# dhansmair/flamingo-mini

Measured on AMD Instinct MI355X. Metric: images/sec (fwd+bwd) flamingo-mini bs=32, higher is better.
Workload: dtype bf16

## Files before the change

### flamingo-mini_amd/build.py

```python
from __future__ import annotations

import concurrent.futures
import os
import shutil
import subprocess
import sys

PKG_DIR = os.path.dirname(os.path.abspath(__file__))
CSRC = os.path.join(PKG_DIR, "csrc")
LIB_PATH = os.path.join(PKG_DIR, "libflamingo_fusion.so")
SOURCES = ["ff_api.hip", "ff_gemm.hip", "ff_rowwise.hip", "ff_attention.hip", "ff_xattn_fused.hip", "ff_optim.hip", "ff_loss.hip", "ff_elementwise.hip", "ff_decode.hip", "ff_sample.hip", "ff_beam.hip", "ff_logits.hip", "ff_logprob.hip", "ff_constrain.hip", "ff_guidance.hip", "ff_truncate.hip", "ff_score.hip", "ff_beam_sample.hip", "ff_contrastive.hip"]
HEADERS = ["ff_common.h", "ff_internal.h", "ff_gemm_tiles.h", "ff_attention_core.h", "ff_row_keys.h", "ff_sr.h", "ff_beam_walk.h", os.path.join("..", "..", "include", "flamingo_fusion.h")]
ARCH = "gfx950"
FLAGS = [f"--offload-arch={ARCH}", "-O3", "-std=c++17", "-fPIC", "-fvisibility=hidden", "-Wno-unused-result", "-mllvm", "-amdgpu-kernarg-preload-count=16"] + os.environ.get("FF_EXTRA_FLAGS", "").split()


def _hipcc() -> str:
    for cand in (os.environ.get("HIPCC"), "/opt/rocm/bin/hipcc", shutil.which("hipcc")):
        if cand and os.path.exists(cand):
            return cand
    raise RuntimeError("hipcc not found (needs ROCm >= 7.0 for gfx950)")


def _stale(target: str, deps) -> bool:
    if not os.path.exists(target):
        return True
    t = os.path.getmtime(target)
    return any(os.path.getmtime(d) > t for d in deps)


def build(force: bool = False, verbose: bool = False, debug: bool = False) -> str:
    hipcc = _hipcc()
    obj_dir = os.path.join(CSRC, "_obj_debug" if debug else "_obj")
    lib_path = LIB_PATH.replace(".so", "_debug.so") if debug else LIB_PATH
    flags = FLAGS + (["-DFF_DEBUG"] if debug else [])
    os.makedirs(obj_dir, exist_ok=True)
    headers = [os.path.normpath(os.path.join(CSRC, h)) for h in HEADERS]
    jobs = []
    for src in SOURCES:
        s = os.path.join(CSRC, src)
        o = os.path.join(obj_dir, src.replace(".hip", ".o"))
        if force or _stale(o, [s] + headers) or not os.path.exists(o.replace(".o", ".resources.txt")):
            jobs.append((s, o))

    def compile_one(job):
        s, o = job
        cmd = [hipcc] + flags + ["-Rpass-analysis=kernel-resource-usage", "-c", s, "-o", o]
        r = subprocess.run(cmd, capture_output=True, text=True)
        if r.returncode != 0:
            raise RuntimeError(f"hipcc failed for {s}:\n{r.stderr[-4000:]}")
        with open(o.replace(".o", ".resources.txt"), "w") as f:
            f.write("\n".join(l for l in r.stderr.splitlines() if "kernel-resource-usage" in l) + "\n")
        if verbose:
            print("compiled", os.path.basename(s))
        return o

    with concurrent.futures.ThreadPoolExecutor(max_workers=len(SOURCES)) as ex:
        list(ex.map(compile_one, jobs))
    objs = [os.path.join(obj_dir, s.replace(".hip", ".o")) for s in SOURCES]
    if force or jobs or _stale(lib_path, objs + [os.path.join(CSRC, "exports.map")]):
        r = subprocess.run([hipcc, f"--offload-arch={ARCH}", "-shared", "-fPIC", f"-Wl,--version-script={os.path.join(CSRC, 'exports.map')}", "-o", lib_path] + objs,
                           capture_output=True, text=True)
        if r.returncode != 0:
            raise RuntimeError(f"link failed:\n{r.stderr[-4000:]}")
# ... 8 lines not shown
```

### flamingo-mini_amd/ffi.py

```python
from __future__ import annotations

import ctypes as C
import os
from typing import Optional, Sequence

import torch

PKG_DIR = os.path.dirname(os.path.abspath(__file__))
_which = os.environ.get("FLAMINGO_FUSION_LIB", "")
LIB_PATH = os.path.join(PKG_DIR, "libflamingo_fusion_debug.so") if _which == "debug" else (_which or os.path.join(PKG_DIR, "libflamingo_fusion.so"))
ABI_VERSION = 6

FF_OK = 0
DTYPE_F32, DTYPE_BF16 = 0, 1
ACT_NONE, ACT_GELU, ACT_SQRELU, ACT_RELU = -1, 0, 1, 2
ACTS = {"gelu": ACT_GELU, "sqrelu": ACT_SQRELU, "relu": ACT_RELU}
ATTN_DENSE, ATTN_MEDIA = 0, 1
RESAMPLER_GLOBAL_PARAMS, RESAMPLER_LAYER_PARAMS, XATTN_PARAMS = 4, 12, 11
XA_SAVED = {"mean_a": 0, "rstd_a": 1, "yn": 2, "y1": 3, "mean_f": 4, "rstd_f": 5, "xn_f": 6}
XA_SAVED_STAGES = {"Qs": 7, "lse": 8, "O": 9, "attn_out": 10, "Hpre": 11, "Aact": 12, "ffw_out": 13}
XA_SAVED_ORDER = ("mean_a", "rstd_a", "yn", "Qs", "lse", "O", "attn_out", "y1", "mean_f", "rstd_f", "xn_f", "Hpre", "Aact", "ffw_out")
XA_STASH = {"dy1": 0, "dH": 1, "dQs": 2}
WGRAD_GROUP_MAX = 12

# ... 81 lines not shown
    _fields_ = [(n, C.c_int) for n in ("dtype", "b", "k", "dim")] + [("ld_hidden", C.c_longlong)] + \
               [(n, C.c_int) for n in ("max_len", "eos", "pad", "reserved")] + \
               [(n, C.c_void_p) for n in ("hidden", "hist", "mask", "cand_tok", "cand_logp", "finished", "next_tok", "logprob", "sel_row", "beam_idx", "score")]


_P, _SZ, _I = C.c_void_p, C.c_size_t, C.c_int
_SIGNATURES = {
    "ff_version": (_I, []),
    "ff_arch": (C.c_char_p, []),
    "ff_last_error": (C.c_char_p, []),
    "ff_gemm_workspace_bytes": (_SZ, [C.POINTER(GemmDesc)]),
    "ff_gemm": (_I, [C.POINTER(GemmDesc), _P, _P, _P, _P, _P, _P, _P, _P, _SZ, _P]),
    "ff_gemm_profile_enable": (_I, [_I]),
    "ff_gemm_profile_read": (_I, [C.POINTER(GemmProfileRecord), _I]),
    "ff_gemm_plan": (_I, [C.POINTER(GemmDesc), C.POINTER(_I), C.POINTER(_I), C.POINTER(_I)]),
    "ff_layernorm_fwd": (_I, [C.POINTER(LnDesc), _P, _P, _P, _P, _P, _P, _P, _P]),
    "ff_layernorm_bwd_workspace_bytes": (_SZ, [C.POINTER(LnDesc)]),
    "ff_layernorm_bwd": (_I, [C.POINTER(LnDesc), _P, _P, _P, _P, _P, _P, _P, _P, _P, _P, _P, _SZ, _P]),
    "ff_rows_reduce_workspace_bytes": (_SZ, [C.POINTER(ReduceDesc)]),
    "ff_rows_reduce": (_I, [C.POINTER(ReduceDesc), _P, _P, _P, _SZ, _P]),
    "ff_gate_grad_workspace_bytes": (_SZ, [_I, _I]),
    "ff_gate_grad": (_I, [_I, _I, _I, _P, _P, _P, _P, _P, _SZ, _P]),
    "ff_text_time": (_I, [_I, _I, _P, _I, _P, _P]),
    "ff_attention_fwd": (_I, [C.POINTER(AttnDesc), _P, _P, _P, _P, _P, _P, _P]),
    "ff_attention_bwd_workspace_bytes": (_SZ, [C.POINTER(AttnDesc)]),
    "ff_attention_bwd": (_I, [C.POINTER(AttnDesc), _P, _P, _P, _P, _P, _P, _P, _P, _P, _P, _P, _SZ, _P]),
    "ff_resampler_saved_bytes": (_SZ, [C.POINTER(ResamplerDesc)]),
    "ff_resampler_scratch_bytes": (_SZ, [C.POINTER(ResamplerDesc)]),
    "ff_resampler_fwd": (_I, [C.POINTER(ResamplerDesc), _P, _P, _P, _P, _SZ, _P, _SZ, _P]),
    "ff_resampler_bwd": (_I, [C.POINTER(ResamplerDesc), _P, _P, _P, _P, _SZ, _P, _P, _P, _SZ, _P]),
    "ff_resampler_prologue_saved_bytes": (_SZ, [C.POINTER(ResamplerDesc)]),
    "ff_resampler_layer_saved_bytes": (_SZ, [C.POINTER(ResamplerDesc)]),
    "ff_resampler_layer_scratch_bytes": (_SZ, [C.POINTER(ResamplerDesc)]),
    "ff_resampler_epilogue_saved_bytes": (_SZ, [C.POINTER(ResamplerDesc)]),
    "ff_resampler_prologue_fwd": (_I, [C.POINTER(ResamplerDesc), _P, _P, _P, _SZ, _P]),
    "ff_resampler_layer_fwd": (_I, [C.POINTER(ResamplerDesc), _P, _P, _P, _SZ, _P, _I, _P, _P, _P, _SZ, _P, _SZ, _P]),
    "ff_resampler_epilogue_fwd": (_I, [C.POINTER(ResamplerDesc), _P, _P, _P, _P, _P, _SZ, _P]),
    "ff_resampler_epilogue_bwd": (_I, [C.POINTER(ResamplerDesc), _P, _P, _P, _P, _SZ, _P, _P, _P, _P, _SZ, _P]),
    "ff_resampler_layer_bwd": (_I, [C.POINTER(ResamplerDesc), _P, _P, _P, _SZ, _P, _I, _P, _P, _P, _SZ, _P, _P, _P, _I, _P, _SZ, _P]),
    "ff_resampler_prologue_bwd": (_I, [C.POINTER(ResamplerDesc), _P, _P, _P, _P, _P, _SZ, _P]),
    "ff_xattn_sync_bytes": (_SZ, []),
    "ff_xattn_sync_status": (_I, [_P, _P]),
    "ff_xattn_saved_bytes": (_SZ, [C.POINTER(XattnDesc)]),
    "ff_xattn_scratch_bytes": (_SZ, [C.POINTER(XattnDesc)]),
    "ff_xattn_kv_offset": (_SZ, [C.POINTER(XattnDesc)]),
    "ff_xattn_saved_view": (_I, [C.POINTER(XattnDesc), _I, C.POINTER(_SZ), C.POINTER(_SZ)]),
    "ff_xattn_block_fwd": (_I, [C.POINTER(XattnDesc), _P, _P, _P, _P, _P, _P, _P, _P, _SZ, _P, _SZ, _P]),
    "ff_quick_gelu_fwd": (_I, [_I, C.c_longlong, _P, _P, _P]),
    "ff_quick_gelu_bwd": (_I, [_I, C.c_longlong, _P, _P, _P, _P]),
    "ff_shifted_ce_fwd": (_I, [_I, _I, _I, _I, _P, _P, C.c_longlong, _P, _P, _P]),
    "ff_shifted_ce_bwd": (_I, [_I, _I, _I, _I, _P, _P, C.c_longlong, _P, _P, _P, _P]),
    "ff_shifted_ce_fwd_reg": (_I, [_I, _I, _I, _I, _P, _P, C.c_longlong, _P, _P, C.c_float, C.c_float, _P]),
    "ff_shifted_ce_bwd_reg": (_I, [_I, _I, _I, _I, _P, _P, C.c_longlong, _P, _P, _P, C.c_float, C.c_float, _P]),
    "ff_adamw_step": (_I, [C.POINTER(AdamWDesc), _P, _P, _P, _P, _P, _P]),
    "ff_adamw_step_mixed": (_I, [C.POINTER(AdamWDesc), _I, _P, _P, _P, _P, _P, _P, _P, _P]),
    "ff_adamw_step_clipped": (_I, [C.POINTER(AdamWDesc), _I, _P, _P, _P, _P, _P, _P, _P, _P, _P]),
    "ff_grad_sumsq_partials": (C.c_longlong, [_I, _P]),
    "ff_grad_sumsq": (_I, [_I, _I, _P, _P, C.c_float, _P, C.c_longlong, _P]),
    "ff_grad_sumsq_reduce": (_I, [_P, C.c_longlong, _P, _I, _P]),
    "ff_grad_clip_coef": (_I, [_P, C.c_float, _P, _P, _P]),
    "ff_scale_grads": (_I, [_I, _I, _P, _P, _P, _P]),
    "ff_grad_accumulate": (_I, [_I, _I, _P, _P, _P, C.c_float, _I, _P]),
    "ff_adamw_step_acc": (_I, [C.POINTER(AdamWDesc), _I, _P, _P, _P, _P, _P, _P, _P, _P, _P]),
    "ff_grad_guard": (_I, [_P, C.c_float, _P, _P, _P, _P, _P, _P, _P, _P]),
    "ff_adamw_step_guarded": (_I, [C.POINTER(AdamWDesc), _I, _P, _P, _I, _P, _P, _P, _P, _P, _P, _P, _P]),
    "ff_adamw_step_sr": (_I, [C.POINTER(AdamWDesc), _I, _P, _P, _I, _P, _P, _P, _P, _P, C.c_longlong, _P, _P, _P]),
    "ff_stochastic_round_bf16": (_I, [_P, _P, C.c_longlong, C.c_longlong, C.c_uint, C.c_uint, _I, _P]),
    "ff_ema_update": (_I, [_I, _I, _P, _P, _P, _P, C.c_float, _I, _I, _I, _P, _P, _P]),
    "ff_sample_token": (_I, [_I, _I, _I, C.c_longlong, _P, C.c_float, _I, C.c_float, _P, _P, _P]),
    "ff_sample_token_truncated": (_I, [_I, _I, _I, C.c_longlong, _P, C.c_float, _I, C.c_float, C.c_float, C.c_float, C.c_float, C.c_float, _P, _P, _P]),
    "ff_beam_workspace_bytes": (_SZ, [_I, _I]),
    "ff_beam_step": (_I, [C.POINTER(BeamDesc), _P, _P, _P, _SZ, _P]),
    "ff_beam_gather": (_I, [_I, _P, _I, _I, _I, C.c_longlong, C.c_longlong, C.c_longlong, _P, _P, _P]),
    "ff_group_beam_step": (_I, [C.POINTER(BeamDesc), _I, C.c_float, _P, _P, _P, _SZ, _P]),
    "ff_beam_sample_workspace_bytes": (_SZ, [_I, _I]),
    "ff_beam_sample_step": (_I, [C.POINTER(BeamDesc), C.c_float, _I, C.c_float, _P, _P, _P, _P, _SZ, _P]),
    "ff_beam_sample_noise": (_I, [_I, _I, _P, _P, _P, _P]),
    "ff_topk_logprob": (_I, [_I, _I, _I, C.c_longlong, _P, _I, _P, _P, _P]),
    "ff_contrastive_step": (_I, [C.POINTER(ContrastiveDesc), _P, _P, _P]),
    "ff_logits_process": (_I, [_I, _I, _I, C.c_longlong, _P, _P, C.c_longlong, C.c_longlong, _P, C.c_float, _I, _I, _P, _P]),
    "ff_token_logprob": (_I, [_I, _I, _I, C.c_longlong, _P, _P, _P, _P, _P, _P]),
    "ff_logprob_gather": (_I, [_I, _I, _I, C.c_longlong, _P, _P, _P, _I, _P, _P, _P]),
    "ff_logits_constrain": (_I, [_I, _I, _I, C.c_longlong, _P, _P, C.c_longlong, C.c_longlong, _P, _P, _I, _P, _P, _P, _P, _P, _I, _I, _P, _P, _P, _I, _I, _P]),
    "ff_guided_logits": (_I, [_I, _I, _I, C.c_longlong, _P, C.c_longlong, _P, _P, _P, C.c_longlong, _P]),
    "ff_xattn_block_bwd_kv": (_I, [C.POINTER(XattnDesc), _P, _P, _P, _P, _P, _P, _P, _SZ, _P, _P, _P, _P, _SZ, _P]),
    "ff_kv_project_workspace_bytes": (_SZ, [C.POINTER(KvProjDesc), _I]),
    "ff_kv_project_fwd": (_I, [C.POINTER(KvProjDesc), _P, _P, _P, _P, _SZ, _P]),
    "ff_kv_project_bwd": (_I, [C.POINTER(KvProjDesc), _P, _P, _P, _P, _P, _P, _SZ, _P]),
    "ff_xattn_wgrad_stash_bytes": (_SZ, [C.POINTER(XattnDesc)]),
    "ff_xattn_wgrad_stash_view": (_I, [C.POINTER(XattnDesc), _I, C.POINTER(_SZ), C.POINTER(_SZ)]),
    "ff_xattn_wgrad_workspace_bytes": (_SZ, [C.POINTER(XattnDesc)]),
    "ff_xattn_block_bwd_kv_data": (_I, [C.POINTER(XattnDesc), _P, _P, _P, _P, _P, _P, _P, _SZ, _P, _P, _P, _P, _SZ, _P, _SZ, _P]),
    "ff_xattn_wgrad_grouped": (_I, [C.POINTER(XattnDesc), _I, _P, _P, _SZ, _P, _SZ, _P, _P, _P, _SZ, _P]),
    "ff_xattn_block_bwd": (_I, [C.POINTER(XattnDesc), _P, _P, _P, _P, _P, _P, _SZ, _P, _P, _P, _P, _SZ, _P]),
}
EXPORTED_SYMBOLS = tuple(_SIGNATURES)

_lib: Optional[C.CDLL] = None


def lib() -> C.CDLL:
    global _lib
    if _lib is not None:
        return _lib
    if not os.path.exists(LIB_PATH):
        raise FusionLibraryError(
# ... 63 lines not shown
```

### flamingo-mini_amd/functional.py

```python
from __future__ import annotations

from typing import Callable, Optional, Sequence, Tuple

import torch

from . import ffi

_grad_ready_callbacks: list = []


def _new(shape, dtype, device) -> torch.Tensor:
    return torch.empty(shape, dtype=dtype, device=device)


def _new_zeros(shape, dtype, device) -> torch.Tensor:
    return torch.zeros(shape, dtype=dtype, device=device)


def _new_like(t: torch.Tensor, dtype=None) -> torch.Tensor:
    return torch.empty_like(t, dtype=dtype)


def _new_zeros_like(t: torch.Tensor, dtype=None) -> torch.Tensor:
    return torch.zeros_like(t, dtype=dtype)
# ... 735 lines not shown
        else:
            ffi.check(lib.ff_shifted_ce_fwd_reg(ffi.dtype_code(logits.dtype), b, L, V, logits.data_ptr(), labels.data_ptr(), ignore_index,
                                                rows.data_ptr(), lse.data_ptr(), label_smoothing, z_loss, ffi.stream_handle(logits.device)),
                      "ff_shifted_ce_fwd_reg")
        ctx.ignore_index, ctx.label_smoothing, ctx.z_loss = ignore_index, label_smoothing, z_loss
        ctx.save_for_backward(logits, labels, lse)
        return rows

    @staticmethod
    def backward(ctx, grad_rows):
        lib = ffi.lib()
        logits, labels, lse = ctx.saved_tensors
        b, L, V = logits.shape
        phase = logits.data_ptr() % 16 // logits.element_size()
        if phase:
            dlogits = _new(logits.numel() + 16 // logits.element_size(), logits.dtype, logits.device)[phase:phase + logits.numel()].view(b, L, V)
        else:
            dlogits = _new_like(logits)
        g = grad_rows.contiguous().float()
        if ctx.label_smoothing == 0.0 and ctx.z_loss == 0.0:
            ffi.check(lib.ff_shifted_ce_bwd(ffi.dtype_code(logits.dtype), b, L, V, logits.data_ptr(), labels.data_ptr(), ctx.ignore_index,
                                            lse.data_ptr(), g.data_ptr(), dlogits.data_ptr(), ffi.stream_handle(logits.device)), "ff_shifted_ce_bwd")
        else:
            ffi.check(lib.ff_shifted_ce_bwd_reg(ffi.dtype_code(logits.dtype), b, L, V, logits.data_ptr(), labels.data_ptr(), ctx.ignore_index,
                                                lse.data_ptr(), g.data_ptr(), dlogits.data_ptr(), ctx.label_smoothing, ctx.z_loss,
                                                ffi.stream_handle(logits.device)), "ff_shifted_ce_bwd_reg")
        return dlogits, None, None, None, None


def check_loss_regularisers(label_smoothing, z_loss) -> Tuple[float, float]:
    eps, zl = float(label_smoothing), float(z_loss)
    if not 0.0 <= eps <= 1.0:
        raise ValueError(f"label_smoothing must lie in [0, 1], got {label_smoothing!r}")
    if not 0.0 <= zl < float("inf"):
        raise ValueError(f"z_loss must be >= 0 and finite, got {z_loss!r}")
    return eps, zl


def shifted_cross_entropy(logits: torch.Tensor, labels: torch.Tensor, reduction: str = "mean", ignore_index: int = -100,
                          label_smoothing: float = 0.0, z_loss: float = 0.0) -> torch.Tensor:
    eps, zl = check_loss_regularisers(label_smoothing, z_loss)
    ffi.require_cuda(logits, labels)
    rows = _ShiftedCEFn.apply(logits, labels, ignore_index, eps, zl)
    if reduction == "none":
        return rows
    if reduction == "sum":
        return rows.sum()
    if reduction == "mean":
        count = (labels[..., 1:] != ignore_index).sum()
        return rows.sum() / count
    raise ValueError(f"unknown reduction {reduction}")


def sample_tokens(logits: torch.Tensor, u: torch.Tensor, temperature: float = 1.0, top_k: int = 0, top_p: float = 1.0,
                  out: Optional[torch.Tensor] = None, *, min_p: float = 0.0, typical_p: float = 1.0, epsilon_cutoff: float = 0.0,
                  eta_cutoff: float = 0.0) -> torch.Tensor:
    ffi.require_cuda(logits, u, out)
    if logits.ndim != 2 or (logits.shape[1] > 1 and logits.stride(1) != 1):
        raise ValueError(f"sample_tokens: logits must be (rows, V) with a contiguous last dimension, got shape {tuple(logits.shape)} strides {logits.stride()}")
    rows, V = logits.shape
    if u.dtype != torch.float32 or u.numel() != rows or not u.is_contiguous():
        raise ValueError(f"sample_tokens: u must be {rows} contiguous float32 values, got {tuple(u.shape)} {u.dtype}")
    if out is None:
        out = _new((rows,), torch.long, logits.device)
    elif out.dtype != torch.long or out.shape != (rows,) or not out.is_contiguous():
        raise ValueError(f"sample_tokens: out must be {rows} contiguous int64 values, got {tuple(out.shape)} {out.dtype}")
    ld = logits.stride(0) if rows > 1 else V
    if min_p == 0 and typical_p == 1 and epsilon_cutoff == 0 and eta_cutoff == 0:
        ffi.check(ffi.lib().ff_sample_token(ffi.dtype_code(logits.dtype), rows, V, ld, logits.data_ptr(), float(temperature), int(top_k), float(top_p),
                                            u.data_ptr(), out.data_ptr(), ffi.stream_handle(logits.device)), "ff_sample_token")
    else:
        ffi.check(ffi.lib().ff_sample_token_truncated(ffi.dtype_code(logits.dtype), rows, V, ld, logits.data_ptr(), float(temperature), int(top_k), float(top_p),
                                                      float(min_p), float(typical_p), float(epsilon_cutoff), float(eta_cutoff),
                                                      u.data_ptr(), out.data_ptr(), ffi.stream_handle(logits.device)), "ff_sample_token_truncated")
    return out


def process_logits(logits: torch.Tensor, hist: torch.Tensor, hist_len: torch.Tensor, repetition_penalty: float = 1.0, no_repeat_ngram_size: int = 0,
                   eos: Optional[int] = None, min_len: Optional[torch.Tensor] = None) -> torch.Tensor:
    ffi.require_cuda(logits, hist, hist_len, min_len)
    if logits.ndim != 2 or (logits.shape[1] > 1 and logits.stride(1) != 1):
        raise ValueError(f"process_logits: logits must be (rows, V) with a contiguous last dimension, got shape {tuple(logits.shape)} strides {logits.stride()}")
    rows, V = logits.shape
    if hist.dtype != torch.long or hist.ndim != 2 or hist.shape[0] != rows or (hist.shape[1] > 1 and hist.stride(1) != 1):
        raise ValueError(f"process_logits: hist must be ({rows}, cap) int64 with a contiguous last dimension, got {tuple(hist.shape)} {hist.dtype} strides {hist.stride()}")
    if hist_len.dtype != torch.long or hist_len.numel() != 1 or (min_len is not None and (min_len.dtype != torch.long or min_len.numel() != 1)):
        raise ValueError("process_logits: hist_len and min_len must each be one int64 value on the device")
    cap = hist.shape[1]
    ffi.check(ffi.lib().ff_logits_process(ffi.dtype_code(logits.dtype), rows, V, logits.stride(0) if rows > 1 else V, logits.data_ptr(),
                                          hist.data_ptr(), hist.stride(0) if rows > 1 else cap, cap, hist_len.data_ptr(), float(repetition_penalty),
                                          int(no_repeat_ngram_size), -1 if eos is None else int(eos), ffi.ptr(min_len), ffi.stream_handle(logits.device)),
              "ff_logits_process")
    return logits


def constrain_logits(logits: torch.Tensor, hist: torch.Tensor, hist_len: torch.Tensor, gen_start: torch.Tensor, eos: Optional[int] = None,
                     trie=None, bad_words=None) -> torch.Tensor:
    tables = tuple(trie or ()) + tuple(bad_words or ())
    ffi.require_cuda(logits, hist, hist_len, gen_start, *tables)
    if logits.ndim != 2 or (logits.shape[1] > 1 and logits.stride(1) != 1):
        raise ValueError(f"constrain_logits: logits must be (rows, V) with a contiguous last dimension, got shape {tuple(logits.shape)} strides {logits.stride()}")
    rows, V = logits.shape
    if hist.dtype != torch.long or hist.ndim != 2 or hist.shape[0] != rows or (hist.shape[1] > 1 and hist.stride(1) != 1):
        raise ValueError(f"constrain_logits: hist must be ({rows}, cap) int64 with a contiguous last dimension, got {tuple(hist.shape)} {hist.dtype} strides {hist.stride()}")
    if any(t.dtype != torch.long or t.numel() != 1 for t in (hist_len, gen_start)):
        raise ValueError("constrain_logits: hist_len and gen_start must each be one int64 value on the device")
# ... 385 lines not shown
```

### flamingo-mini_amd/modeling_flamingo.py

```python
from __future__ import annotations

import contextlib
import logging
from abc import ABC, abstractmethod
from typing import Any, Dict, List, Optional

import torch
import torch.nn as nn
import torch.nn.functional as TF
from transformers import PreTrainedModel
from transformers.modeling_outputs import CausalLMOutputWithPast

from . import decoding as D
from . import functional as F
from .backbones import load_language_model, load_vision_encoder
from .configuration_flamingo import FlamingoConfig
from .decoding import _DecodeSession, _beam_finalize, _repeat_leading
from .gated_cross_attention import ModifiedLMBlock
from .perceiver_resampler import PerceiverResampler
from .utils import get_common_prefix_length


@contextlib.contextmanager
def suppress_model_loading_warnings(suppress: bool = True):
# ... 60 lines not shown
            del self._kv_group_before_cuts
        for i, hook in enumerate(self.get_modified_layers()):
            hook.autograd_cut = cuts.cut if (cuts is not None and i > 0 and i % max(1, segment_layers) == 0) else None
        self.resampler.autograd_cut = cuts.cut if (cuts is not None and getattr(self.resampler, "layerwise", False)) else None

    def _init_weights(self, module):
        pass

    def _init_layers(self, lm_layers: nn.ModuleList):
        c = self.config
        for i in range(0, len(lm_layers), c.xattn_every):
            lm_layers[i] = ModifiedLMBlock(
                lm_layers[i], dim=c.dim, dim_visual=c.dim_visual, dim_head=c.xattn_dim_head, heads=c.xattn_heads,
                ff_mult=c.xattn_ff_mult, act=c.xattn_act, n_visual=c.resampler_num_latents)

    @abstractmethod
    def get_modified_layers(self) -> List[ModifiedLMBlock]:
        raise NotImplementedError

    def freeze_vm(self):
        self.vision_encoder.requires_grad_(False)

    def freeze_lm(self):
        self.lm.requires_grad_(False)
        self.lm.get_input_embeddings().weight.requires_grad = True
        for hook in self.get_modified_layers():
            hook.xattn_block.requires_grad_(True)

    def unfreeze_lm(self):
        self.lm.requires_grad_(True)

    def state_dict_trainable(self) -> Dict[str, torch.Tensor]:
        names = {n for n, p in self.named_parameters() if p.requires_grad}
        return {k: v for k, v in self.state_dict().items() if k in names}

    def parameters_trainable(self):
        return (p for p in self.parameters() if p.requires_grad)

    def encode_resample_visuals(self, pixel_values: torch.Tensor) -> torch.Tensor:
        if pixel_values.ndim == 4:
            b, N, T = 1, pixel_values.size(0), 1
        elif pixel_values.ndim == 5:
            b, N, T = pixel_values.size(0), pixel_values.size(1), 1
        elif pixel_values.ndim == 6:
            b, N, T = pixel_values.shape[:3]
        else:
            raise ValueError("pixel_values must have ndim 5 or 6!")
        frames = pixel_values.reshape(b * N * T, *pixel_values.shape[-3:])
        with torch.no_grad():
            feats = self.vision_encoder(frames).last_hidden_state
        feats = feats.reshape(b * N, T, feats.shape[-2], feats.shape[-1])
        latents = self.resampler(feats)
        return latents.reshape(b, N, latents.shape[-2], latents.shape[-1])

    def forward(self, input_ids=None, attention_mask=None, media_locations=None, pixel_values=None, visual_features=None,
                head_mask=None, inputs_embeds=None, use_cache: bool = False, past_key_values=None, return_dict: bool = True,
                labels=None, loss_reduction: str = "mean", text_time=None, label_smoothing: Optional[float] = None,
                z_loss: Optional[float] = None, output_last_hidden_state: bool = False, **kwargs) -> CausalLMOutputWithPast:
        assert return_dict, "can only use return_dict=True at the moment!"
        eps, zeta = F.check_loss_regularisers(getattr(self.config, "label_smoothing", 0.0) if label_smoothing is None else label_smoothing,
                                              getattr(self.config, "z_loss", 0.0) if z_loss is None else z_loss)
        assert (input_ids is None) != (inputs_embeds is None), "you must pass either input_ids or inputs_embeds!"
        ref = input_ids if input_ids is not None else inputs_embeds
        batch_size, seq_length = ref.shape[:2]
        device = ref.device
        xattn_past = None if past_key_values is None else past_key_values[0]
        lm_past = None if past_key_values is None else past_key_values[1]

        if visual_features is None:
            if xattn_past is None and pixel_values is not None:
                assert pixel_values.size(0) == batch_size, "pixel_values must have the same batch size as the textual input!"
                visual_features = self.encode_resample_visuals(pixel_values)
            else:
                visual_features = torch.zeros((batch_size, 1, self.config.resampler_num_latents, self.config.dim_visual),
                                              dtype=self.resampler.latents.dtype, device=device)
        if self.training and (getattr(self.lm, "gradient_checkpointing", False) or any(getattr(m, "gradient_checkpointing", False) for m in self.lm.modules())):
            raise NotImplementedError("activation checkpointing of the language model is not supported by the fused cross-attention hooks: "
                                      "their conditioning (visual features, hoisted K / V) is released when forward() returns. "
                                      "Disable gradient checkpointing (the frozen LM keeps few activations: only the trainable blocks save theirs).")
        if self.training and device.type == "cuda" and not torch.cuda.is_current_stream_capturing():
            F.poll_sync_exchange("FlamingoBaseModel.forward")
        cuts = getattr(self, "_autograd_cuts", None)
        if cuts is not None and xattn_past is None:
            visual_features = cuts.cut(visual_features)
        if text_time is None:
            if media_locations is None:
                media_locations = torch.zeros((batch_size, seq_length), dtype=torch.int, device=device)
            text_time = F.text_time(media_locations)
        hooks = self.get_modified_layers()
        hoisted = None
        if xattn_past is None and self.hoist_kv:
            weights = [h.xattn_block.attn.to_kv.weight for h in hooks]
            cdt = F.autocast_compute_dtype(visual_features)
            if cdt is not None:
                weights = F.autocast_params(weights, cdt)
            vf_cast = visual_features.to(weights[0].dtype)
            step = self.kv_project_group if self.kv_project_group > 0 else len(weights)
            hoisted = [kv for g in range(0, len(weights), step) for kv in F.kv_project(vf_cast, weights[g:g + step])]
        for i, hook in enumerate(hooks):
            hook.condition(visual_features, media_locations, None if xattn_past is None else xattn_past[i], text_time=text_time,
                           hoisted_kv=None if hoisted is None else hoisted[i])

        lm_kwargs = dict(input_ids=input_ids, attention_mask=attention_mask, inputs_embeds=inputs_embeds, use_cache=use_cache,
                         past_key_values=lm_past, return_dict=True, **kwargs)
        if head_mask is not None:
            lm_kwargs["head_mask"] = head_mask
        try:
            out = self.lm(**lm_kwargs)
        finally:
            for hook in hooks:
                hook.condition(None, None)
        logits = self.lm_head(out.last_hidden_state)

        new_xattn_past = [hook.kv_output for hook in hooks] if use_cache else None
        for hook in hooks:
            hook.kv_output = None

        loss = None
        if labels is not None:
            if logits.is_cuda and logits.dtype in (torch.float32, torch.bfloat16) and logits.ndim == 3 and seq_length > 1:
                loss = F.shifted_cross_entropy(logits, labels, reduction=loss_reduction, label_smoothing=eps, z_loss=zeta)
            else:
                flat = logits[..., :-1, :].contiguous().view(-1, logits.size(-1))
                if flat.dtype in (torch.bfloat16, torch.float16):
                    flat = flat.float()
                target = labels[..., 1:].contiguous().view(-1)
                if eps == 0.0 and zeta == 0.0:
                    loss = TF.cross_entropy(flat, target, reduction=loss_reduction)
                else:
                    rows = TF.cross_entropy(flat, target, reduction="none", label_smoothing=eps)
                    if zeta != 0.0:
                        rows = rows + torch.where(target != -100, zeta * torch.logsumexp(flat, dim=-1).square(), torch.zeros_like(rows))
                    if loss_reduction == "none":
                        loss = rows
                    elif loss_reduction == "sum":
                        loss = rows.sum()
                    elif loss_reduction == "mean":
                        loss = rows.sum() / (target != -100).sum()
                    else:
                        raise ValueError(f"unknown reduction {loss_reduction}")

        return CausalLMOutputWithPast(
            loss=loss, logits=logits,
            past_key_values=(tuple(new_xattn_past), out.past_key_values) if use_cache else None,
            hidden_states=(out.last_hidden_state,) if output_last_hidden_state else getattr(out, "hidden_states", None), attentions=getattr(out, "attentions", None))


class FlamingoGPT2(FlamingoBaseModel):
    _tied_weights_keys = {"lm_head.weight": "lm.wte.weight"}
    lm_family = "gpt2"

    def __init__(self, config: FlamingoConfig):
        assert config.lm.startswith("gpt")
        super().__init__(config)
        base_lm = load_language_model(config)
        assert config.dim == base_lm.config.n_embd, \
            f"specified {config.dim=} in FlamingoConfig, but {config.lm} has hidden size={base_lm.config.n_embd}"
        _add_eoc_row(base_lm)
        self.lm = base_lm.transformer
        self.lm_head = base_lm.lm_head
        self._init_layers(self.lm.h)
        self.post_init()

    def get_modified_layers(self):
        return [layer for layer in self.lm.h if isinstance(layer, ModifiedLMBlock)]


class FlamingoOPT(FlamingoBaseModel):
    _tied_weights_keys = {"lm_head.weight": "lm.decoder.embed_tokens.weight"}
    lm_family = "opt"

    def __init__(self, config: FlamingoConfig):
# ... 317 lines not shown
```

### include/flamingo_fusion.h

```cpp
#ifndef FLAMINGO_FUSION_H
#define FLAMINGO_FUSION_H

#include <stddef.h>

#ifdef __cplusplus
extern "C" {
#endif
#if defined(__GNUC__) || defined(__clang__)
#pragma GCC visibility push(default)
#endif

typedef struct ihipStream_t* ff_stream_t;

enum { FF_OK = 0, FF_ERR_SHAPE = -1, FF_ERR_UNSUPPORTED = -2, FF_ERR_WORKSPACE = -3, FF_ERR_LAUNCH = -4 };
enum { FF_DTYPE_F32 = 0, FF_DTYPE_BF16 = 1 };
enum { FF_ACT_NONE = -1, FF_ACT_GELU = 0, FF_ACT_SQRELU = 1, FF_ACT_RELU = 2 };

int ff_version(void);
const char* ff_arch(void);
const char* ff_last_error(void);

typedef struct ff_rowmap {
    long long ld;
    long long seg_stride;
// ... 179 lines not shown

typedef struct ff_adamw_desc {
    int dtype;
    int n_tensors;
    int step;
    float lr, beta1, beta2, eps, weight_decay, grad_scale;
    const float* step_dev;
} ff_adamw_desc;
int ff_adamw_step(const ff_adamw_desc* d, void* const* params, const void* const* grads, void* const* exp_avg,
                  void* const* exp_avg_sq, const long long* numels, ff_stream_t stream);
int ff_adamw_step_mixed(const ff_adamw_desc* d, int state_dtype, void* const* params, const void* const* grads, void* const* exp_avg,
                        void* const* exp_avg_sq, float* const* master, const float* lr_dev, const long long* numels, ff_stream_t stream);
int ff_adamw_step_clipped(const ff_adamw_desc* d, int state_dtype, void* const* params, const void* const* grads, void* const* exp_avg,
                          void* const* exp_avg_sq, float* const* master, const float* lr_dev, const float* grad_coef, const long long* numels,
                          ff_stream_t stream);

long long ff_grad_sumsq_partials(int n_tensors, const long long* numels);
int ff_grad_sumsq(int dtype, int n_tensors, const void* const* grads, const long long* numels, float scale, float* partials,
                  long long n_partials, ff_stream_t stream);
int ff_grad_sumsq_reduce(const float* partials, long long n_partials, double* sum, int accumulate, ff_stream_t stream);
int ff_grad_clip_coef(const double* sum, float max_norm, float* norm, float* coef, ff_stream_t stream);
int ff_scale_grads(int dtype, int n_tensors, void* const* grads, const long long* numels, const float* coef, ff_stream_t stream);

int ff_grad_accumulate(int dtype, int n_tensors, const void* const* grads, float* const* acc, const long long* numels, float scale,
                       int overwrite, ff_stream_t stream);
int ff_adamw_step_acc(const ff_adamw_desc* d, int state_dtype, void* const* params, const float* const* grads32, void* const* exp_avg,
                      void* const* exp_avg_sq, float* const* master, const float* lr_dev, const float* grad_coef, const long long* numels,
                      ff_stream_t stream);

int ff_grad_guard(const double* sum, float max_norm, const float* ext_found_inf, const float* ext_scale, float* norm, float* coef,
                  float* skip, float* take, long long* skipped_total, ff_stream_t stream);
int ff_adamw_step_guarded(const ff_adamw_desc* d, int state_dtype, void* const* params, const void* const* grads, int grads_fp32,
                          void* const* exp_avg, void* const* exp_avg_sq, float* const* master, const float* lr_dev, const float* grad_coef,
                          const float* skip, const long long* numels, ff_stream_t stream);

int ff_adamw_step_sr(const ff_adamw_desc* d, int state_dtype, void* const* params, const void* const* grads, int grads_fp32,
                     void* const* exp_avg, void* const* exp_avg_sq, const float* lr_dev, const float* grad_coef, const float* skip,
                     long long seed, const unsigned* stream_ids, const long long* numels, ff_stream_t stream);
int ff_stochastic_round_bf16(const float* src, void* dst, long long n, long long seed, unsigned stream_id, unsigned step, int slot,
                             ff_stream_t stream);

int ff_ema_update(int dtype, int n_tensors, const void* const* params, const float* const* master, float* const* ema,
                  const long long* numels, float decay, int warmup, int every, int step, const float* step_dev,
                  const float* skip, ff_stream_t stream);

int ff_shifted_ce_fwd(int dtype, int batch, int seq, int vocab, const void* logits, const long long* labels, long long ignore_index,
                      float* loss_row, float* lse, ff_stream_t stream);
int ff_shifted_ce_bwd(int dtype, int batch, int seq, int vocab, const void* logits, const long long* labels, long long ignore_index,
                      const float* lse, const float* grad_row, void* dlogits, ff_stream_t stream);
int ff_shifted_ce_fwd_reg(int dtype, int batch, int seq, int vocab, const void* logits, const long long* labels, long long ignore_index,
                          float* loss_row, float* lse, float label_smoothing, float z_loss, ff_stream_t stream);
int ff_shifted_ce_bwd_reg(int dtype, int batch, int seq, int vocab, const void* logits, const long long* labels, long long ignore_index,
                          const float* lse, const float* grad_row, void* dlogits, float label_smoothing, float z_loss, ff_stream_t stream);

int ff_sample_token(int dtype, int rows, int vocab, long long ld, const void* logits, float temperature, int top_k, float top_p,
                    const float* u, long long* token, ff_stream_t stream);

int ff_sample_token_truncated(int dtype, int rows, int vocab, long long ld, const void* logits, float temperature, int top_k, float top_p,
                              float min_p, float typical_p, float epsilon_cutoff, float eta_cutoff, const float* u, long long* token,
                              ff_stream_t stream);

#define FF_BEAM_MAX 8
struct ff_beam_desc {
    int dtype, b, nb, vocab;
    long long ld;
    int max_len, eos, pad, early_stopping;
    float* score;
    int* done;
    int* n_hyp;
    float* hyp_score;
    int* hyp_len;
    int* hyp_row;
    long long* hist_tok;
    int* hist_parent;
    float* hist_score;
    long long* next_tok;
    long long* beam_idx;
    const float* len_norm;
};
typedef struct ff_beam_desc ff_beam_desc;
size_t ff_beam_workspace_bytes(int b, int nb);
int ff_beam_step(const ff_beam_desc* d, const void* logits, const long long* cur_len, void* workspace, size_t workspace_bytes,
                 ff_stream_t stream);
int ff_beam_gather(int n_tensors, void* const* tensors, int elem_size, int b, int nb, long long outer, long long len_max, long long inner,
                   const long long* beam_idx, const long long* n_pos, ff_stream_t stream);

int ff_group_beam_step(const ff_beam_desc* d, int n_groups, float diversity_penalty, const void* logits, const long long* cur_len,
                       void* workspace, size_t workspace_bytes, ff_stream_t stream);

size_t ff_beam_sample_workspace_bytes(int b, int nb);
int ff_beam_sample_step(const ff_beam_desc* d, float temperature, int top_k, float top_p, const long long* seed, const void* logits,
                        const long long* cur_len, void* workspace, size_t workspace_bytes, ff_stream_t stream);
int ff_beam_sample_noise(int rows, int vocab, const long long* seed, const long long* cur_len, float* g, ff_stream_t stream);

#define FF_CONTRASTIVE_K_MAX 8
struct ff_contrastive_desc {
    int dtype, b, k, dim;
    long long ld_hidden;
    int max_len, eos, pad, reserved;
    const void* hidden;
    void* hist;
    const unsigned char* mask;
    const long long* cand_tok;
    const float* cand_logp;
    unsigned char* finished;
    long long* next_tok;
// ... 43 lines not shown
```

Baseline: 802.3.

## Fuse LM head projection with shifted CE and padded-stride dlogits backward

Routes the LM head plus shifted cross-entropy through a custom autograd function. Its backward writes dlogits into a buffer whose row stride is padded to a multiple of 8 elements, then feeds that buffer straight into the d_hidden and d_weight GEMMs. The aim is to avoid a separate logits-gradient pass through autograd and to give the GEMMs aligned leading dimensions when the vocab size is odd. In exchange it adds a new kernel, an extra padded buffer, and a possible add of grad_logits when the logits output is also used downstream.

```diff
diff --git a/flamingo-mini_amd/build.py b/flamingo-mini_amd/build.py
--- a/flamingo-mini_amd/build.py
+++ b/flamingo-mini_amd/build.py
@@ -9,7 +9,7 @@
 PKG_DIR = os.path.dirname(os.path.abspath(__file__))
 CSRC = os.path.join(PKG_DIR, "csrc")
 LIB_PATH = os.path.join(PKG_DIR, "libflamingo_fusion.so")
-SOURCES = ["ff_api.hip", "ff_gemm.hip", "ff_rowwise.hip", "ff_attention.hip", "ff_xattn_fused.hip", "ff_optim.hip", "ff_loss.hip", "ff_elementwise.hip", "ff_decode.hip", "ff_sample.hip", "ff_beam.hip", "ff_logits.hip", "ff_logprob.hip", "ff_constrain.hip", "ff_guidance.hip", "ff_truncate.hip", "ff_score.hip", "ff_beam_sample.hip", "ff_contrastive.hip"]
+SOURCES = ["ff_api.hip", "ff_gemm.hip", "ff_rowwise.hip", "ff_attention.hip", "ff_xattn_fused.hip", "ff_optim.hip", "ff_loss.hip", "ff_elementwise.hip", "ff_decode.hip", "ff_sample.hip", "ff_beam.hip", "ff_logits.hip", "ff_logprob.hip", "ff_constrain.hip", "ff_guidance.hip", "ff_truncate.hip", "ff_score.hip", "ff_beam_sample.hip", "ff_contrastive.hip", "ff_lm_head.hip"]
 HEADERS = ["ff_common.h", "ff_internal.h", "ff_gemm_tiles.h", "ff_attention_core.h", "ff_row_keys.h", "ff_sr.h", "ff_beam_walk.h", os.path.join("..", "..", "include", "flamingo_fusion.h")]
 ARCH = "gfx950"
 FLAGS = [f"--offload-arch={ARCH}", "-O3", "-std=c++17", "-fPIC", "-fvisibility=hidden", "-Wno-unused-result", "-mllvm", "-amdgpu-kernarg-preload-count=16"] + os.environ.get("FF_EXTRA_FLAGS", "").split()
diff --git a/flamingo-mini_amd/csrc/ff_lm_head.hip b/flamingo-mini_amd/csrc/ff_lm_head.hip
--- /dev/null
+++ b/flamingo-mini_amd/csrc/ff_lm_head.hip
@@ -0,0 +1,76 @@
+#include "ff_common.h"
+
+namespace ff {
+
+template <typename T> struct __attribute__((packed, aligned(sizeof(T)))) UnalignedVec { typename Vec<T>::raw v; };
+
+template <typename T, typename... Reg>
+__global__ __launch_bounds__(256) void lm_head_dlogits_kernel(int L, int V, const T* __restrict__ logits, const long long* __restrict__ labels,
+                                                              long long ignore_index, const float* __restrict__ lse, const float* __restrict__ g,
+                                                              T* __restrict__ dlogits, long long ld, Reg... reg) {
+    constexpr bool REG = sizeof...(Reg) == 2;
+    static_assert(REG || sizeof...(Reg) == 0, "lm_head_dlogits_kernel: no trailing argument, or eps and zl");
+    pin_args(L, V, logits, labels, ignore_index, lse, g, dlogits, ld, reg...);
+    const int b = blockIdx.x / L, i = blockIdx.x - b * L;
+    constexpr int N = Vec<T>::N;
+    const T* row = logits + ((long long)b * L + i) * V;
+    T* drow = dlogits + ((long long)b * L + i) * ld;
+    const bool last = i == L - 1;
+    const int r = b * (L - 1) + i;
+    const long long tgt = last ? -1 : labels[(long long)b * L + i + 1];
+    const float gr = (last || tgt == ignore_index) ? 0.f : ((tgt < 0 || tgt >= V) ? __builtin_nanf("") : g[r]), l = last ? 0.f : lse[r];
+    const float ez[3] = {reg..., 0.f}, pk = 1.f + 2.f * ez[1] * l, sgn = pk < 0.f ? -1.f : 1.f, lk = l - logf(fabsf(pk));
+    const float hot = 1.f - ez[0], eov = ez[0] / (float)V;
+    auto dval = [&](int c, float x) {
+        if constexpr (!REG) return gr == 0.f ? 0.f : (__expf(x - l) - (c == tgt ? 1.f : 0.f)) * gr;
+        else return gr == 0.f ? 0.f : (__expf(x - lk) * sgn - (c == tgt ? hot : 0.f) - eov) * gr;
+    };
+    const int nvec = (int)(ld / N);
+    for (int v = threadIdx.x; v < nvec; v += 256) {
+        const int c0 = v * N;
+        float x[N];
+        if (c0 + N <= V) {
+            const typename Vec<T>::raw q = ((const UnalignedVec<T>*)(row + c0))->v;
+#pragma unroll
+            for (int e = 0; e < N; e++) x[e] = dval(c0 + e, to_f32((T)q[e]));
+        } else {
+#pragma unroll
+            for (int e = 0; e < N; e++) x[e] = c0 + e < V ? dval(c0 + e, to_f32(row[c0 + e])) : 0.f;
+        }
+        Vec<T>::store(drow + c0, x);
+    }
+}
+
+}
+
+extern "C" int ff_shifted_ce_bwd_reg_ld(int dtype, int batch, int seq, int vocab, const void* logits, const long long* labels, long long ignore_index,
+                                        const float* lse, const float* grad_row, void* dlogits, long long ld_dlogits, float label_smoothing,
+                                        float z_loss, ff_stream_t stream) {
+    using namespace ff;
+    FF_CHECK(batch > 0 && seq > 1 && vocab > 0 && logits && labels && lse && grad_row && dlogits, FF_ERR_SHAPE, "ff_shifted_ce_bwd_ld: bad arguments");
+    FF_CHECK(label_smoothing >= 0.f && label_smoothing <= 1.f && z_loss >= 0.f && z_loss <= 3.402823466e+38f, FF_ERR_UNSUPPORTED,
+             "ff_shifted_ce_bwd_reg_ld: label_smoothing %g must lie in [0, 1], z_loss %g be >= 0 and finite", (double)label_smoothing, (double)z_loss);
+    FF_CHECK(dtype == FF_DTYPE_BF16 || dtype == FF_DTYPE_F32, FF_ERR_UNSUPPORTED, "ff_shifted_ce_bwd_ld: dtype %d", dtype);
+    const long long per16 = 16 / (long long)dtype_size(dtype);
+    FF_CHECK(ld_dlogits >= vocab && ld_dlogits % per16 == 0, FF_ERR_UNSUPPORTED,
+             "ff_shifted_ce_bwd_ld: ld_dlogits %lld must be >= vocab %d and a multiple of %lld elements (16 bytes)", ld_dlogits, vocab, per16);
+    FF_CHECK(ld_dlogits < (1LL << 31), FF_ERR_UNSUPPORTED, "ff_shifted_ce_bwd_ld: ld_dlogits %lld must be below 2^31", ld_dlogits);
+    FF_CHECK(((unsigned long long)dlogits & 15u) == 0, FF_ERR_UNSUPPORTED, "ff_shifted_ce_bwd_ld: dlogits must be 16-byte aligned");
+    FF_CHECK(((unsigned long long)logits % dtype_size(dtype)) == 0, FF_ERR_UNSUPPORTED, "ff_shifted_ce_bwd_ld: logits must be element-aligned");
+    const dim3 grid(batch * seq);
+    hipStream_t st = (hipStream_t)stream;
+    if (label_smoothing == 0.f && z_loss == 0.f) {
+        if (dtype == FF_DTYPE_BF16) lm_head_dlogits_kernel<bf16><<<grid, dim3(256), 0, st>>>(seq, vocab, (const bf16*)logits, labels, ignore_index, lse, grad_row, (bf16*)dlogits, ld_dlogits);
+        else lm_head_dlogits_kernel<float><<<grid, dim3(256), 0, st>>>(seq, vocab, (const float*)logits, labels, ignore_index, lse, grad_row, (float*)dlogits, ld_dlogits);
+    } else if (dtype == FF_DTYPE_BF16) {
+        lm_head_dlogits_kernel<bf16><<<grid, dim3(256), 0, st>>>(seq, vocab, (const bf16*)logits, labels, ignore_index, lse, grad_row, (bf16*)dlogits, ld_dlogits, label_smoothing, z_loss);
+    } else {
+        lm_head_dlogits_kernel<float><<<grid, dim3(256), 0, st>>>(seq, vocab, (const float*)logits, labels, ignore_index, lse, grad_row, (float*)dlogits, ld_dlogits, label_smoothing, z_loss);
+    }
+    return check_launch("lm_head_dlogits");
+}
+
+extern "C" int ff_shifted_ce_bwd_ld(int dtype, int batch, int seq, int vocab, const void* logits, const long long* labels, long long ignore_index,
+                                    const float* lse, const float* grad_row, void* dlogits, long long ld_dlogits, ff_stream_t stream) {
+    return ff_shifted_ce_bwd_reg_ld(dtype, batch, seq, vocab, logits, labels, ignore_index, lse, grad_row, dlogits, ld_dlogits, 0.f, 0.f, stream);
+}
diff --git a/flamingo-mini_amd/ffi.py b/flamingo-mini_amd/ffi.py
--- a/flamingo-mini_amd/ffi.py
+++ b/flamingo-mini_amd/ffi.py
@@ -157,6 +157,8 @@
     "ff_shifted_ce_bwd": (_I, [_I, _I, _I, _I, _P, _P, C.c_longlong, _P, _P, _P, _P]),
     "ff_shifted_ce_fwd_reg": (_I, [_I, _I, _I, _I, _P, _P, C.c_longlong, _P, _P, C.c_float, C.c_float, _P]),
     "ff_shifted_ce_bwd_reg": (_I, [_I, _I, _I, _I, _P, _P, C.c_longlong, _P, _P, _P, C.c_float, C.c_float, _P]),
+    "ff_shifted_ce_bwd_ld": (_I, [_I, _I, _I, _I, _P, _P, C.c_longlong, _P, _P, _P, C.c_longlong, _P]),
+    "ff_shifted_ce_bwd_reg_ld": (_I, [_I, _I, _I, _I, _P, _P, C.c_longlong, _P, _P, _P, C.c_longlong, C.c_float, C.c_float, _P]),
     "ff_adamw_step": (_I, [C.POINTER(AdamWDesc), _P, _P, _P, _P, _P, _P]),
     "ff_adamw_step_mixed": (_I, [C.POINTER(AdamWDesc), _I, _P, _P, _P, _P, _P, _P, _P, _P]),
     "ff_adamw_step_clipped": (_I, [C.POINTER(AdamWDesc), _I, _P, _P, _P, _P, _P, _P, _P, _P, _P]),
diff --git a/flamingo-mini_amd/functional.py b/flamingo-mini_amd/functional.py
--- a/flamingo-mini_amd/functional.py
+++ b/flamingo-mini_amd/functional.py
@@ -811,6 +811,81 @@
     raise ValueError(f"unknown reduction {reduction}")
 
 
+lm_head_fused_backward = True
+lm_head_ce_calls = 0
+
+
+def lm_head_ce_applicable(hidden: torch.Tensor, weight: torch.Tensor) -> bool:
+    return (hidden.is_cuda and hidden.dtype == torch.bfloat16 and weight.dtype == torch.bfloat16 and weight.device == hidden.device and
+            hidden.ndim == 3 and weight.ndim == 2 and hidden.shape[1] > 1 and hidden.shape[2] == weight.shape[1] and weight.shape[1] % 8 == 0)
+
+
+class _LmHeadCEFn(torch.autograd.Function):
+    @staticmethod
+    def forward(ctx, hidden, weight, labels, ignore_index, label_smoothing, z_loss):
+        lib = ffi.lib()
+        logits = torch.nn.functional.linear(hidden, weight)
+        labels = labels.contiguous().to(torch.int64)
+        b, L, V = logits.shape
+        rows = _new(b * (L - 1), torch.float32, logits.device)
+        lse = _new_like(rows)
+        if label_smoothing == 0.0 and z_loss == 0.0:
+            ffi.check(lib.ff_shifted_ce_fwd(ffi.dtype_code(logits.dtype), b, L, V, logits.data_ptr(), labels.data_ptr(), ignore_index,
+                                            rows.data_ptr(), lse.data_ptr(), ffi.stream_handle(logits.device)), "ff_shifted_ce_fwd")
+        else:
+            ffi.check(lib.ff_shifted_ce_fwd_reg(ffi.dtype_code(logits.dtype), b, L, V, logits.data_ptr(), labels.data_ptr(), ignore_index,
+                                                rows.data_ptr(), lse.data_ptr(), label_smoothing, z_loss, ffi.stream_handle(logits.device)),
+                      "ff_shifted_ce_fwd_reg")
+        ctx.ignore_index, ctx.label_smoothing, ctx.z_loss = ignore_index, label_smoothing, z_loss
+        ctx.save_for_backward(hidden, weight, logits, labels, lse)
+        return logits, rows
+
+    @staticmethod
+    def backward(ctx, grad_logits, grad_rows):
+        lib = ffi.lib()
+        hidden, weight, logits, labels, lse = ctx.saved_tensors
+        b, L, V = logits.shape
+        dim = weight.shape[1]
+        ld = (V + 7) // 8 * 8
+        dl = _new((b * L, ld), logits.dtype, logits.device)
+        stream = ffi.stream_handle(logits.device)
+        g = (grad_rows if grad_rows is not None else _new_zeros(b * (L - 1), torch.float32, logits.device)).contiguous().float()
+        if ctx.label_smoothing == 0.0 and ctx.z_loss == 0.0:
+            ffi.check(lib.ff_shifted_ce_bwd_ld(ffi.dtype_code(logits.dtype), b, L, V, logits.data_ptr(), labels.data_ptr(), ctx.ignore_index,
+                                               lse.data_ptr(), g.data_ptr(), dl.data_ptr(), ld, stream), "ff_shifted_ce_bwd_ld")
+        else:
+            ffi.check(lib.ff_shifted_ce_bwd_reg_ld(ffi.dtype_code(logits.dtype), b, L, V, logits.data_ptr(), labels.data_ptr(), ctx.ignore_index,
+                                                   lse.data_ptr(), g.data_ptr(), dl.data_ptr(), ld, ctx.label_smoothing, ctx.z_loss, stream),
+                      "ff_shifted_ce_bwd_reg_ld")
+        if grad_logits is not None:
+            dl[:, :V].add_(grad_logits.reshape(b * L, V))
+        d_hidden = d_weight = None
+        if ctx.needs_input_grad[0]:
+            d_hidden = torch.mm(dl[:, :V], weight).view(b, L, dim)
+        if ctx.needs_input_grad[1]:
+            d_weight = torch.mm(dl[:, :V].t(), hidden.reshape(b * L, dim))
+        return d_hidden, d_weight, None, None, None, None
+
+
+def lm_head_shifted_ce(hidden: torch.Tensor, weight: torch.Tensor, labels: torch.Tensor, reduction: str = "mean", ignore_index: int = -100,
+                       label_smoothing: float = 0.0, z_loss: float = 0.0) -> Tuple[torch.Tensor, torch.Tensor]:
+    global lm_head_ce_calls
+    eps, zl = check_loss_regularisers(label_smoothing, z_loss)
+    ffi.require_cuda(hidden, weight, labels)
+    if not lm_head_ce_applicable(hidden, weight):
+        raise ffi.FusionLibraryError("lm_head_shifted_ce needs bfloat16 hidden (b, L > 1, dim) and weight (V, dim) on one GPU with dim % 8 == 0")
+    if reduction not in ("none", "sum", "mean"):
+        raise ValueError(f"unknown reduction {reduction}")
+    lm_head_ce_calls += 1
+    logits, rows = _LmHeadCEFn.apply(hidden, weight, labels, ignore_index, eps, zl)
+    if reduction == "none":
+        return logits, rows
+    if reduction == "sum":
+        return logits, rows.sum()
+    count = (labels[..., 1:] != ignore_index).sum()
+    return logits, rows.sum() / count
+
+
 def sample_tokens(logits: torch.Tensor, u: torch.Tensor, temperature: float = 1.0, top_k: int = 0, top_p: float = 1.0,
                   out: Optional[torch.Tensor] = None, *, min_p: float = 0.0, typical_p: float = 1.0, epsilon_cutoff: float = 0.0,
                   eta_cutoff: float = 0.0) -> torch.Tensor:
diff --git a/flamingo-mini_amd/modeling_flamingo.py b/flamingo-mini_amd/modeling_flamingo.py
--- a/flamingo-mini_amd/modeling_flamingo.py
+++ b/flamingo-mini_amd/modeling_flamingo.py
@@ -136,6 +136,12 @@
         feats = feats.reshape(b * N, T, feats.shape[-2], feats.shape[-1])
         latents = self.resampler(feats)
         return latents.reshape(b, N, latents.shape[-2], latents.shape[-1])
+
+    def _lm_head_ce_route(self, hidden: torch.Tensor, labels, seq_length: int) -> bool:
+        head = self.lm_head
+        return (F.lm_head_fused_backward and labels is not None and torch.is_grad_enabled() and seq_length > 1
+                and type(head) is nn.Linear and head.bias is None and not head._forward_hooks and not head._forward_pre_hooks
+                and F.autocast_compute_dtype(hidden) is None and F.lm_head_ce_applicable(hidden, head.weight))
 
     def forward(self, input_ids=None, attention_mask=None, media_locations=None, pixel_values=None, visual_features=None,
                 head_mask=None, inputs_embeds=None, use_cache: bool = False, past_key_values=None, return_dict: bool = True,
@@ -194,14 +200,18 @@
         finally:
             for hook in hooks:
                 hook.condition(None, None)
-        logits = self.lm_head(out.last_hidden_state)
+        loss = None
+        if self._lm_head_ce_route(out.last_hidden_state, labels, seq_length):
+            logits, loss = F.lm_head_shifted_ce(out.last_hidden_state, self.lm_head.weight, labels, reduction=loss_reduction,
+                                                label_smoothing=eps, z_loss=zeta)
+        else:
+            logits = self.lm_head(out.last_hidden_state)
 
         new_xattn_past = [hook.kv_output for hook in hooks] if use_cache else None
         for hook in hooks:
             hook.kv_output = None
 
-        loss = None
-        if labels is not None:
+        if labels is not None and loss is None:
             if logits.is_cuda and logits.dtype in (torch.float32, torch.bfloat16) and logits.ndim == 3 and seq_length > 1:
                 loss = F.shifted_cross_entropy(logits, labels, reduction=loss_reduction, label_smoothing=eps, z_loss=zeta)
             else:
diff --git a/include/flamingo_fusion.h b/include/flamingo_fusion.h
--- a/include/flamingo_fusion.h
+++ b/include/flamingo_fusion.h
@@ -255,6 +255,11 @@
                           float* loss_row, float* lse, float label_smoothing, float z_loss, ff_stream_t stream);
 int ff_shifted_ce_bwd_reg(int dtype, int batch, int seq, int vocab, const void* logits, const long long* labels, long long ignore_index,
                           const float* lse, const float* grad_row, void* dlogits, float label_smoothing, float z_loss, ff_stream_t stream);
+int ff_shifted_ce_bwd_ld(int dtype, int batch, int seq, int vocab, const void* logits, const long long* labels, long long ignore_index,
+                         const float* lse, const float* grad_row, void* dlogits, long long ld_dlogits, ff_stream_t stream);
+int ff_shifted_ce_bwd_reg_ld(int dtype, int batch, int seq, int vocab, const void* logits, const long long* labels, long long ignore_index,
+                             const float* lse, const float* grad_row, void* dlogits, long long ld_dlogits, float label_smoothing, float z_loss,
+                             ff_stream_t stream);
 
 int ff_sample_token(int dtype, int rows, int vocab, long long ld, const void* logits, float temperature, int top_k, float top_p,
                     const float* u, long long* token, ff_stream_t stream);
```

Result: no change. 799.9 (-0.3%).
